# slbouknight/accelerated-ray-tracer

Measured on AMD Instinct MI355X. Metric: Mrays/s, 1200x800 random scene @ 500 spp (frame ms in ms_per_step), higher is better.
Workload: dtype f32

## Files before the change

accelerated-ray-tracer_amd/__init__.py:

```python
from __future__ import annotations

import collections
import ctypes as C
import os
import subprocess

import numpy as np

PKG_DIR = os.path.dirname(os.path.realpath(__file__))
REPO_ROOT = os.path.dirname(PKG_DIR)
LIB_DIR = os.path.join(PKG_DIR, "lib")
RT_LIB_PATH = os.environ.get("RT_LIB_OVERRIDE") or os.path.join(LIB_DIR, "librt_mi355x.so")
HOST_LIB_PATH = os.environ.get("RTW_LIB_OVERRIDE") or os.path.join(LIB_DIR, "librtw_host.so")


class RtError(RuntimeError):
    pass


class RtCamera(C.Structure):
    _fields_ = [("origin", C.c_float * 3), ("lower_left_corner", C.c_float * 3), ("horizontal", C.c_float * 3),
                ("vertical", C.c_float * 3), ("u", C.c_float * 3), ("v", C.c_float * 3), ("lens_radius", C.c_float),
                ("pad", C.c_float), ("time0", C.c_double), ("time1", C.c_double)]

# ... 497 lines not shown
        except Exception:
            pass


def _frame_buffers(color):
    bufs = _Buffers(isinstance(color, np.ndarray), "color", _initialised_device)
    if not (bufs.on_host or hasattr(color, "data_ptr")):
        raise bufs.wrong_kind("color", "a numpy array")
    if color.ndim != 3 or color.shape[2] != 3 or color.shape[0] < 1 or color.shape[1] < 1:
        raise ValueError(f"color: shape {tuple(color.shape)}, expected (ny, nx, 3)")
    ny, nx = int(color.shape[0]), int(color.shape[1])
    if nx * ny >= 1 << 31:
        raise ValueError("frame too large")
    return bufs, nx, ny


_initialised_device = None


def init(device: int = 0) -> None:
    global _initialised_device
    _check(rt_lib().rt_init(device), "rt_init")
    _initialised_device = device


def set_option(key: str, value: int) -> None:
    _check(rt_lib().rt_set_option(key.encode(), int(value)), f"rt_set_option({key})")


def reset_options() -> None:
    _check(rt_lib().rt_reset_options(), "rt_reset_options")


def denoise_workspace_bytes(nx: int, ny: int) -> int:
    return int(rt_lib().rt_denoise_workspace_bytes(int(nx), int(ny)))


def denoise(color, albedo=None, normal=None, depth=None, *, iterations=DENOISE_DEFAULTS["iterations"],
            sigma_color=None, color_floor=DENOISE_DEFAULTS["color_floor"],
            normal_sharpness=DENOISE_DEFAULTS["normal_sharpness"], sigma_depth=DENOISE_DEFAULTS["sigma_depth"], demodulate=None,
            out=None, workspace=None, stream=0, blocking=True, variance=None, variance_out=None,
            sigma_variance=DENOISE_VARIANCE_DEFAULTS["sigma_variance"], variance_floor=DENOISE_VARIANCE_DEFAULTS["variance_floor"]):
    if variance is None:
        if variance_out is not None:
            raise ValueError("variance_out needs variance")
        if sigma_color is None:
            sigma_color = DENOISE_DEFAULTS["sigma_color"]
    else:
        if sigma_color is not None and float(sigma_color) != 0:
            raise ValueError("sigma_color must be left out or 0 with a variance: the variance factor replaces the colour factor")
        sigma_color = 0.0
        sigma_variance, variance_floor = float(sigma_variance), float(variance_floor)
        if not (np.isfinite(sigma_variance) and np.float32(1e-6) <= np.float32(sigma_variance) <= np.float32(1e6)):
            raise ValueError("sigma_variance must be in [1e-6, 1e6]")
        if not (np.isfinite(variance_floor) and 0 < np.float32(variance_floor) < np.inf):
            raise ValueError("variance_floor must be finite and positive")
    bufs, nx, ny = _frame_buffers(color)
    for k, v, lo, hi in (("iterations", iterations, 1, 8), ("normal_sharpness", normal_sharpness, 0, 10)):
        if isinstance(v, bool) or not isinstance(v, (int, np.integer)) or not lo <= int(v) <= hi:
            raise ValueError(f"{k} must be an integer in {lo}..{hi}")
    sigma_color, color_floor, sigma_depth = float(sigma_color), float(color_floor), float(sigma_depth)
    for k, v in (("sigma_color", sigma_color), ("sigma_depth", sigma_depth)):
        if not (v == 0 or (np.isfinite(v) and np.float32(1e-6) <= np.float32(v) <= np.float32(1e6))):
            raise ValueError(f"{k} must be 0 or in [1e-6, 1e6]")
    if sigma_color > 0 and not (np.isfinite(color_floor) and 0 < np.float32(color_floor) < np.inf):
        raise ValueError("color_floor must be finite and positive")
# ... 349 lines not shown
    def spheres(self) -> np.ndarray:
        out = np.zeros(self.host.desc.n_spheres, SPHERE_DTYPE)
        _check(rt_lib().rt_scene_get_spheres(self._p, out.ctypes.data, len(out)), "rt_scene_get_spheres")
        return out

    def instances(self) -> np.ndarray:
        out = np.zeros(self.host.desc.n_instances, INSTANCE_DTYPE)
        _check(rt_lib().rt_scene_get_instances(self._p, out.ctypes.data, len(out)), "rt_scene_get_instances")
        return out

    def quads(self) -> np.ndarray:
        out = np.zeros(self.host.desc.n_quads, QUAD_DTYPE)
        _check(rt_lib().rt_scene_get_quads(self._p, out.ctypes.data, len(out)), "rt_scene_get_quads")
        return out

    def debug_quads(self):
        quads, boxes = np.zeros(self.host.desc.n_quads, QUAD_DTYPE), np.zeros(self.host.desc.n_boxes, np.int32)
        _check(rt_lib().rt_debug_scene_quads(self._p, quads.ctypes.data if len(quads) else None, len(quads),
                                             boxes.ctypes.data if len(boxes) else None, len(boxes)), "rt_debug_scene_quads")
        return quads, boxes

    COST_MAP_STATES = ("none", "exact", "stale")

    def cost_map(self):
        L = rt_lib()
        info = (C.c_int32 * 4)()
        _check(L.rt_debug_cost_map(self._p, None, 0, info), "rt_debug_cost_map")
        if info[0] == 0:
            return "none", None, int(info[3])
        out = np.zeros((int(info[2]), int(info[1])), np.uint32)
        _check(L.rt_debug_cost_map(self._p, out.ctypes.data, out.size, info), "rt_debug_cost_map")
        return self.COST_MAP_STATES[info[0]], out, int(info[3])

    def set_cost_map(self, costs) -> None:
        a = np.ascontiguousarray(costs, np.uint32)
        _check(rt_lib().rt_debug_set_cost_map(self._p, a.ctypes.data, a.size), "rt_debug_set_cost_map")

    def render(self, frame: RtFrameDesc, out=None, stream: int = 0, blocking: bool = True):
        L = rt_lib()
        rows = L.rt_frame_local_rows(C.byref(frame))
        if rows < 0:
            raise RtError("bad row partition")
        stats = RtStats()
        if out is None:
            out = np.empty((rows, frame.nx, 3), np.float32)
        if isinstance(out, np.ndarray):
            assert out.dtype == np.float32 and out.size == rows * frame.nx * 3 and out.flags["C_CONTIGUOUS"]
            _check(L.rt_render(self._p, C.byref(frame), out.ctypes.data, 0, stream, 1, C.byref(stats)), "rt_render")
            return out, stats
        _check(L.rt_render(self._p, C.byref(frame), C.c_void_p(int(out)), 1, stream, 1 if blocking else 0, C.byref(stats)), "rt_render")
        return None, stats

    def _ray_buffers(self, origins, directions):
        bufs = _Buffers(isinstance(origins, np.ndarray), "origins", self.device)
        if not (bufs.on_host or hasattr(origins, "data_ptr")):
            raise bufs.wrong_kind("origins", "a numpy array")
        if origins.ndim != 2 or origins.shape[1] != 3:
            raise ValueError(f"origins: shape {tuple(origins.shape)}, expected (N, 3)")
        if directions is None:
            raise ValueError("directions are required")
        return bufs, int(origins.shape[0])

    def trace(self, origins, directions, times=None, tmin: float = 0.001, tmax=None, any_hit: bool = False, record: bool = False,
              stream=None):
        import torch
        if any_hit and record:
# ... 463 lines not shown
```

accelerated-ray-tracer_amd/csrc/rt_abi.hip:

```cpp
#include <hip/hip_runtime.h>

#include <algorithm>
#include <cfloat>
#include <utility>
#include <cmath>
#include <functional>
#include <cstdio>
#include <cstring>
#include <string>
#include <vector>

#include "../../include/rt_abi.h"
#include "rt_call_buffers.h"
#include "rt_device.h"
#include "rt_refit_host.h"

namespace {

struct device_info {
    bool ready = false;
    int num_cu = 256;
    size_t lds_per_cu = 160 * 1024;
};
enum { RT_MAX_DEVICES = 16 };
device_info g_devices[RT_MAX_DEVICES];
int g_device = -1;
int g_last_hip_error = 0;
std::string g_detail;

struct rt_options {
    int kernel = RT_KERNEL_STAGED;
    int lds_mode = -1;
    int steps_per_trip = 12;
    int shade_threshold = 0;
    int wg_per_cu = 0;
    int threads = 0;
    int leaf_threshold = 8;
    int diel_threshold = 2;
    int box_threshold = 8;
    int medium_threshold = 16;
    int newpath_threshold = 0;
    int sparse_stride = 8;
    int split_samples = 16;
    int tier_auto = 1;
    int tier_kernel = 1;
    int prior = 1;
    int resplit_samples = 0;
    int presplit_samples = 0;
    int tier1_factor_x10 = 45;
    int tier1_pixels = 1536;
    int cost_smooth_percent = 0;
    int tier1_depth = 3;
    int heavy_factor_x10 = 20;
    int sparse_factor_x10 = 40;
    int heavy_max_tiles = 0;
    int semi_stride = -1;
    int sparse_priority = 3;
    int tier_priority = 1;
    int semi_priority = 1;
    int handoff = 1;
    int handoff_scan = 1;
    int handoff_poll_us = 1000;
    int handoff_pixels = -1;
    int sparse_eager = 0;
    int sparse_work_percent = 5;
    int sparse_wg_percent = 35;
    int bvh_collapse = 3;
    int scan_nodes = 24;
    int multi_force_rccl = 0;
    int lpt = 1;
    int cost_map = 1;
    int trace_lds = -1;
    int trace_tree = 1;
    int radiance_lds = -1;
    int aov_lds = -1;
    int aov_through_lds = -1;
    int denoise_lds = -1;
    int upscale_lds = -1;
    int adaptive_tier = -1;
};
rt_options g_opt;
unsigned long long g_opt_epoch = 0;

#define HIPCHK(expr)                                                                  \
    do {                                                                              \
        hipError_t e_ = (expr);                                                       \
        if (e_ != hipSuccess) {                                                       \
            g_last_hip_error = (int)e_;                                               \
            char buf_[512];                                                           \
            snprintf(buf_, sizeof(buf_), "HIP error = %u at %s:%d '%s' (%s)", (unsigned)e_, __FILE__, __LINE__, #expr, \
                     hipGetErrorString(e_));                                          \
            g_detail = buf_;                                                          \
            return RT_ERR_HIP;                                                        \
        }                                                                             \
    } while (0)
#define RT_TRY(expr) do { const rt_status st_ = (expr); if (st_ != RT_OK) return st_; } while (0)
// ... 37 lines not shown
        if (guarded && !all.empty()) (void)hipStreamSynchronize(stream);
        for (void* p : all) (void)hipFree(p);
    }
    void guard(hipStream_t st) { stream = st; guarded = true; }
    void settled() { guarded = false; }
    hipError_t get(void** p, size_t bytes) { const hipError_t e = hipMalloc(p, bytes ? bytes : 1); if (e == hipSuccess) all.push_back(*p); return e; }
    rt_status finish(bool wait) { if (wait) HIPCHK(hipStreamSynchronize(stream)); settled(); return RT_OK; }
};

}

rt_status rt_internal_scene_create_on(int device, const rt_scene_desc* d, rt_scene** out);

struct rt_scene {
    int device = 0;
    rt_scene_dev dev;
    std::vector<void*> allocs;
    bool spheres_only = false, need_uv = false;
    int tex_level = 0;
    size_t node_bytes = 0, sphere_bytes = 0, shade_bytes = 0;
    double walk_tests_before = 0, walk_tests_after = 0;
    unsigned long long* d_ray_counter = nullptr;
    unsigned int* d_work_counter = nullptr;
    float* d_fb = nullptr;
    size_t d_fb_floats = 0;
    unsigned int* d_tile_cost = nullptr;
    unsigned int* d_tile_order = nullptr;
    rt_pixel_state* d_state = nullptr;
    unsigned long long* d_heavy_list = nullptr;
    unsigned int* d_heavy_pixels = nullptr;
    size_t tile_capacity = 0, pixel_capacity = 0;
    unsigned long long* d_handoff = nullptr;
    size_t handoff_capacity = 0;
    rt_rank_info* d_rank = nullptr;
    unsigned int* d_cal_cost = nullptr;
    int cal_nx = 0, cal_ny = 0;
    struct cost_map_key {
        int32_t nx = 0, ny = 0, tile_rows = 0, tile_first = 0, tile_stride = 0, local_rows = 0, kernel_variant = 0;
        bool operator==(const cost_map_key& o) const {
            return nx == o.nx && ny == o.ny && tile_rows == o.tile_rows && tile_first == o.tile_first && tile_stride == o.tile_stride &&
                   local_rows == o.local_rows && kernel_variant == o.kernel_variant;
        }
    };
    struct cost_map_state {
        unsigned int* d = nullptr;
        size_t capacity = 0;
        bool valid = false, pending = false;
        cost_map_key key, last_key;
        bool have_last_key = false;
        unsigned long long scene_epoch = 0, opt_epoch = 0, total = 0;
        int last_parts = 0;
    } cost_map;
    unsigned long long scene_epoch = 0;
    hipStream_t tier_stream = nullptr;
    hipEvent_t ev_fork[4] = {nullptr, nullptr, nullptr, nullptr}, ev_join[4] = {nullptr, nullptr, nullptr, nullptr};
    bool ranked_frame = false;
    hipEvent_t ev_start = nullptr, ev_stop = nullptr;
    bool frame_pending = false;
    hipStream_t pending_stream = nullptr;
    rt_stats pending_stats;
    rt_pixel_state* d_adapt_state = nullptr;
    float* d_adapt_half = nullptr;
    uint32_t* d_adapt_list[2] = {nullptr, nullptr};
    unsigned long long* d_adapt_queue = nullptr;
    int32_t* d_adapt_spp = nullptr;
    uint32_t* d_adapt_count = nullptr;
// ... 402 lines not shown

const char* rt_strerror(rt_status s) {
    switch (s) {
    case RT_OK: return "ok";
    case RT_ERR_INVALID: return "invalid argument or malformed scene description";
    case RT_ERR_NO_DEVICE: return "no gfx950 HIP device";
    case RT_ERR_HIP: return "HIP runtime error";
    case RT_ERR_UNSUPPORTED: return "unsupported scene construct";
    default: return "unknown status";
    }
}
int rt_last_hip_error(void) { return g_last_hip_error; }
const char* rt_last_error_detail(void) { return g_detail.c_str(); }

rt_status rt_set_option(const char* key, int value) {
    if (!key) return invalid("null option key");
    ++g_opt_epoch;
    const std::string k(key);
    if (k == "kernel") { if (value != RT_KERNEL_PIXEL && value != RT_KERNEL_STAGED) return invalid("kernel: 0 (pixel) or 3 (staged)"); g_opt.kernel = value; }
    else if (k == "leaf_threshold") { if (value < 1 || value > 64) return invalid("leaf_threshold: 1..64"); g_opt.leaf_threshold = value; }
    else if (k == "box_threshold") { if (value < 1 || value > 64) return invalid("box_threshold: 1..64"); g_opt.box_threshold = value; }
    else if (k == "medium_threshold") { if (value < 1 || value > 64) return invalid("medium_threshold: 1..64"); g_opt.medium_threshold = value; }
    else if (k == "diel_threshold") { if (value < 1 || value > 64) return invalid("diel_threshold: 1..64"); g_opt.diel_threshold = value; }
    else if (k == "newpath_threshold") { if (value < 0 || value > 64) return invalid("newpath_threshold: 0 (by kernel family) or 1..64"); g_opt.newpath_threshold = value; }
    else if (k == "sparse_stride") { if (value != 0 && value != 2 && value != 4 && value != 8 && value != 16 && value != 32 && value != 64) return invalid("sparse_stride: 0, 2, 4, ... 64"); g_opt.sparse_stride = value; }
    else if (k == "sparse_factor_x10") { if (value < 10 || value > 1000) return invalid("sparse_factor_x10: 10..1000"); g_opt.sparse_factor_x10 = value; }
    else if (k == "heavy_factor_x10") { if (value < 10 || value > 1000) return invalid("heavy_factor_x10: 10..1000"); g_opt.heavy_factor_x10 = value; }
    else if (k == "tier_auto") { if (value < 0 || value > 1) return invalid("tier_auto: 0 or 1"); g_opt.tier_auto = value; }
    else if (k == "tier_kernel") { if (value < 0 || value > 1) return invalid("tier_kernel: 0 or 1"); g_opt.tier_kernel = value; }
    else if (k == "handoff") { if (value < 0 || value > 1) return invalid("handoff: 0 or 1"); g_opt.handoff = value; }
    else if (k == "handoff_scan") { if (value < 0 || value > 1) return invalid("handoff_scan: 0 or 1"); g_opt.handoff_scan = value; }
    else if (k == "handoff_poll_us") { if (value < 1 || value > 1000000) return invalid("handoff_poll_us: 1..1000000"); g_opt.handoff_poll_us = value; }
    else if (k == "handoff_pixels") { if (value < -1 || value > (1 << 24)) return invalid("handoff_pixels: -1 (auto) or 0..16777216"); g_opt.handoff_pixels = value; }
    else if (k == "prior") { if (value < 0 || value > 1) return invalid("prior: 0 or 1"); g_opt.prior = value; }
    else if (k == "presplit_samples") { if (value < 0 || value > 4096) return invalid("presplit_samples: 0..4096"); g_opt.presplit_samples = value; }
    else if (k == "resplit_samples") { if (value < 0 || value > 65536) return invalid("resplit_samples: 0..65536"); g_opt.resplit_samples = value; }
    else if (k == "split_samples") { if (value < 1 || value > 4096) return invalid("split_samples: 1..4096"); g_opt.split_samples = value; }
    else if (k == "tier1_factor_x10") { if (value < 10 || value > 10000) return invalid("tier1_factor_x10: 10..10000"); g_opt.tier1_factor_x10 = value; }
    else if (k == "cost_smooth_percent") { if (value < 0 || value > 100) return invalid("cost_smooth_percent: 0..100"); g_opt.cost_smooth_percent = value; }
    else if (k == "tier1_depth") { if (value < 1 || value > 64) return invalid("tier1_depth: 1..64"); g_opt.tier1_depth = value; }
    else if (k == "tier1_pixels") { if (value < 0 || value > 65536) return invalid("tier1_pixels: 0..65536"); g_opt.tier1_pixels = value; }
    else if (k == "semi_stride") { if (value != -1 && value != 0 && value != 1 && value != 2 && value != 4 && value != 8) return invalid("semi_stride: -1 (by kernel family), 0, 1, 2, 4 or 8"); g_opt.semi_stride = value; }
    else if (k == "sparse_eager") { if (value < 0 || value > 1) return invalid("sparse_eager: 0 or 1"); g_opt.sparse_eager = value; }
    else if (k == "tier_priority") { if (value < 0 || value > 3) return invalid("tier_priority: 0..3"); g_opt.tier_priority = value; }
    else if (k == "semi_priority") { if (value < 0 || value > 3) return invalid("semi_priority: 0..3"); g_opt.semi_priority = value; }
    else if (k == "sparse_priority") { if (value < 0 || value > 3) return invalid("sparse_priority: 0..3"); g_opt.sparse_priority = value; }
    else if (k == "sparse_work_percent") { if (value < 0 || value > 100) return invalid("sparse_work_percent: 0..100"); g_opt.sparse_work_percent = value; }
    else if (k == "sparse_wg_percent") { if (value < 1 || value > 100) return invalid("sparse_wg_percent: 1..100"); g_opt.sparse_wg_percent = value; }
    else if (k == "heavy_max_tiles") { if (value < 0 || value > 4096) return invalid("heavy_max_tiles: 0..4096"); g_opt.heavy_max_tiles = value; }
    else if (k == "bvh_collapse") { if (value < 0 || value > 3) return invalid("bvh_collapse: 0..3 (read by rt_scene_create)"); g_opt.bvh_collapse = value; }
    else if (k == "scan_nodes") { if (value < 0 || value > 64) return invalid("scan_nodes: 0..64"); g_opt.scan_nodes = value; }
    else if (k == "multi_force_rccl") { if (value < 0 || value > 1) return invalid("multi_force_rccl: 0 or 1"); g_opt.multi_force_rccl = value; }
    else if (k == "cost_map") { if (value < 0 || value > 1) return invalid("cost_map: 0 or 1"); g_opt.cost_map = value; }
    else if (k == "lpt") { if (value < 0 || value > 1) return invalid("lpt: 0 or 1"); g_opt.lpt = value; }
    else if (k == "threads") { if (value != 0 && (value < 64 || value > 768 || (value % 64))) return invalid("threads: 0 (per kernel family) or a multiple of 64 up to 768 (512 for the lean spheres-only kernels)"); g_opt.threads = value; }
    else if (k == "lds_mode") { if (value < -1 || value > 4) return invalid("lds_mode: -1..4"); g_opt.lds_mode = value; }
    else if (k == "steps_per_trip") { if (value < 1 || value > 64) return invalid("steps_per_trip: 1..64"); g_opt.steps_per_trip = value; }
    else if (k == "shade_threshold") { if (value < 0 || value > 64) return invalid("shade_threshold: 0 (by the launch's load) or 1..64"); g_opt.shade_threshold = value; }
    else if (k == "trace_lds") { if (value < -1 || value > 2) return invalid("trace_lds: -1 (auto) .. 2"); g_opt.trace_lds = value; }
    else if (k == "radiance_lds") { if (value < -1 || value > 2) return invalid("radiance_lds: -1 (auto) .. 2"); g_opt.radiance_lds = value; }
    else if (k == "aov_lds") { if (value < -1 || value > 2) return invalid("aov_lds: -1 (auto) .. 2"); g_opt.aov_lds = value; }
    else if (k == "aov_through_lds") { if (value < -1 || value > 2) return invalid("aov_through_lds: -1 (auto) .. 2"); g_opt.aov_through_lds = value; }
    else if (k == "denoise_lds") { if (value < -1 || value > 1) return invalid("denoise_lds: -1 (auto), 0 (direct) or 1 (staged)"); g_opt.denoise_lds = value; }
    else if (k == "upscale_lds") { if (value < -1 || value > 1) return invalid("upscale_lds: -1 (auto), 0 (direct) or 1 (staged)"); g_opt.upscale_lds = value; }
    else if (k == "trace_tree") { if (value < 0 || value > 1) return invalid("trace_tree: 0 (reference tree) or 1 (walk array)"); g_opt.trace_tree = value; }
    else if (k == "adaptive_tier") { if (value < -1 || value > 1) return invalid("adaptive_tier: -1 (auto), 0 (main kernel) or 1 (tier kernel)"); g_opt.adaptive_tier = value; }
    else if (k == "wg_per_cu") { if (value < 0 || value > 8) return invalid("wg_per_cu: 0 (per kernel family) .. 8"); g_opt.wg_per_cu = value; }
    else return invalid("unknown option");
    return RT_OK;
}

rt_status rt_scene_destroy(rt_scene* s) {
    if (!s) return RT_OK;
    (void)use_device(s->device);
    for (void* p : s->allocs) (void)hipFree(p);
    if (s->d_ray_counter) (void)hipFree(s->d_ray_counter);
    if (s->d_work_counter) (void)hipFree(s->d_work_counter);
    if (s->d_fb) (void)hipFree(s->d_fb);
    if (s->d_tile_cost) (void)hipFree(s->d_tile_cost);
    if (s->d_tile_order) (void)hipFree(s->d_tile_order);
    if (s->d_state) (void)hipFree(s->d_state);
    if (s->d_heavy_list) (void)hipFree(s->d_heavy_list);
    if (s->d_heavy_pixels) (void)hipFree(s->d_heavy_pixels);
    if (s->d_rank) (void)hipFree(s->d_rank);
    if (s->d_handoff) (void)hipFree(s->d_handoff);
    if (s->d_cal_cost) (void)hipFree(s->d_cal_cost);
    if (s->cost_map.d) (void)hipFree(s->cost_map.d);
    for (void* p : {s->refit.block, (void*)s->refit.d_indices, (void*)s->refit.d_records}) if (p) (void)hipFree(p);
    for (void* p : {(void*)s->d_adapt_state, (void*)s->d_adapt_half, (void*)s->d_adapt_list[0], (void*)s->d_adapt_list[1], (void*)s->d_adapt_queue,
                    (void*)s->d_adapt_spp, (void*)s->d_adapt_count, (void*)s->d_adapt_rank, (void*)s->d_var_acc})
        if (p) (void)hipFree(p);
    for (hipEvent_t e : s->adapt_events) (void)hipEventDestroy(e);
    if (s->tier_stream) (void)hipStreamDestroy(s->tier_stream);
    for (int k = 0; k < 4; ++k) { if (s->ev_fork[k]) (void)hipEventDestroy(s->ev_fork[k]); if (s->ev_join[k]) (void)hipEventDestroy(s->ev_join[k]); }
    if (s->ev_start) (void)hipEventDestroy(s->ev_start);
    if (s->ev_stop) (void)hipEventDestroy(s->ev_stop);
    delete s;
    return RT_OK;
}

namespace {
rt_status measure_pass_counts(rt_scene* s, const rt_node* d_tree, int n_tree, std::vector<double>& pass, double& rays, std::vector<float>* sample = nullptr, uint32_t sample_stride = 0, bool keep_cost = false) {
    const rt_camera& c = s->dev.camera;
    const double hw = sqrt((double)c.horizontal[0] * c.horizontal[0] + (double)c.horizontal[1] * c.horizontal[1] + (double)c.horizontal[2] * c.horizontal[2]);
    const double vh = sqrt((double)c.vertical[0] * c.vertical[0] + (double)c.vertical[1] * c.vertical[1] + (double)c.vertical[2] * c.vertical[2]);
    double aspect = (hw > 0 && vh > 0) ? hw / vh : 1.0;
    if (!(aspect > 0.05 && aspect < 20.0)) aspect = 1.0;
    int nx = aspect >= 1.0 ? 256 : (int)(256 * aspect + 0.5), ny = aspect >= 1.0 ? (int)(256 / aspect + 0.5) : 256;
    if (nx < 8) nx = 8;
    if (ny < 8) ny = 8;
    const int n = n_tree;
    rt_scene_dev dev = s->dev;
    dev.nodes_ref = d_tree; dev.n_nodes_ref = n_tree;
    unsigned int* d_pass = nullptr;
    unsigned int* d_cost = nullptr;
    float* d_fb = nullptr;
    HIPCHK(hipMalloc((void**)&d_pass, (size_t)n * sizeof(unsigned int)));
    hipError_t e = hipMalloc((void**)&d_fb, (size_t)nx * ny * 3 * sizeof(float));
// ... 1303 lines not shown
}

rt_status rt_reproject(const rt_reproject_desc* d, int buffers_on_device, void* stream_v, int blocking) {
    return reproject_impl(d, nullptr, nullptr, nullptr, "rt_reproject", buffers_on_device, stream_v, blocking);
}

rt_status rt_reproject_moving(const rt_reproject_desc* d, const rt_reproject_motion_desc* m, int buffers_on_device, void* stream_v, int blocking) {
    if (!m) return invalid("rt_reproject_moving: null motion description");
    return reproject_impl(d, m, nullptr, nullptr, "rt_reproject_moving", buffers_on_device, stream_v, blocking);
}

rt_status rt_reproject_instances(const rt_reproject_desc* d, const rt_reproject_motion_desc* m, const rt_reproject_instance_desc* im,
                                 int buffers_on_device, void* stream_v, int blocking) {
    if (!m) return invalid("rt_reproject_instances: null motion description");
    if (!im) return invalid("rt_reproject_instances: null instance description");
    return reproject_impl(d, m, im, nullptr, "rt_reproject_instances", buffers_on_device, stream_v, blocking);
}

rt_status rt_reproject_quads(const rt_reproject_desc* d, const rt_reproject_motion_desc* m, const rt_reproject_instance_desc* im,
                             const rt_reproject_quad_desc* qm, int buffers_on_device, void* stream_v, int blocking) {
    if (!m) return invalid("rt_reproject_quads: null motion description");
    if (!im) return invalid("rt_reproject_quads: null instance description");
    if (!qm) return invalid("rt_reproject_quads: null quad description");
    return reproject_impl(d, m, im, qm, "rt_reproject_quads", buffers_on_device, stream_v, blocking);
}

rt_status rt_debug_handoff(rt_scene* s, unsigned long long* out2) {
    if (!s || !out2) return invalid("null argument");
    RT_TRY(use_device(s->device));
    HIPCHK(hipMemcpy(out2, s->d_ray_counter + 28, 2 * sizeof(unsigned long long), hipMemcpyDeviceToHost));
    return RT_OK;
}

rt_status rt_debug_counters(rt_scene* s, unsigned long long* out16) {
    if (!s || !out16) return invalid("null argument");
    RT_TRY(use_device(s->device));
    HIPCHK(hipMemcpy(out16, s->d_ray_counter + 1, 16 * sizeof(unsigned long long), hipMemcpyDeviceToHost));
    return RT_OK;
}
rt_status rt_debug_stage_cycles(rt_scene* s, unsigned long long* out10) {
    if (!s || !out10) return invalid("null argument");
    RT_TRY(use_device(s->device));
    HIPCHK(hipMemcpy(out10, s->d_ray_counter + 17, 10 * sizeof(unsigned long long), hipMemcpyDeviceToHost));
    return RT_OK;
}
rt_status rt_debug_wave_ends(rt_scene* s, unsigned long long* out, int n) {
    if (!s || !out || n < 0 || n > 2 * RT_DIAG_BINS) return invalid("bad argument");
    RT_TRY(use_device(s->device));
    HIPCHK(hipMemcpy(out, s->d_ray_counter + RT_DIAG_HIST_SLOT, (size_t)n * sizeof(unsigned long long), hipMemcpyDeviceToHost));
    return RT_OK;
}
rt_status rt_debug_wave_last(rt_scene* s, unsigned long long* out, int n_waves) {
    if (!s || !out || n_waves < 0 || n_waves > RT_DIAG_MAX_WAVES) return invalid("bad argument");
    RT_TRY(use_device(s->device));
    HIPCHK(hipMemcpy(out, s->d_ray_counter + RT_DIAG_WAVE_SLOT, (size_t)2 * n_waves * sizeof(unsigned long long), hipMemcpyDeviceToHost));
    return RT_OK;
}

namespace {
enum { RANK_PARAM_WORDS = 20, RANK_INFO_WORDS = 13 };
static_assert(sizeof(rt_rank_info) == RANK_INFO_WORDS * 4, "rt_debug_rank / rt_debug_rank_info copy rt_rank_info as 13 words");
}

rt_status rt_debug_rank(const uint32_t* cost, const uint32_t* tile_cost, uint64_t rays, const uint32_t* params, uint32_t* tile_order,
                        uint32_t* cost_out, uint32_t* heavy_pixels, uint32_t* info13) {
    if (!cost || !tile_cost || !params || !tile_order || !cost_out || !heavy_pixels || !info13) return invalid("rt_debug_rank: null argument");
// ... 495 lines not shown
    dim3 grid = ml.grid;
    const dim3 block = ml.block;
    const int per_cu_resident = ml.per_cu_resident;

    bool tier_possible = false;
    unsigned tier_grid = 0;
    int tier_waves_per_main_wg = 0;
    tier_room room = {false, 0, 0, 0};
    if (kernel == RT_KERNEL_STAGED && (g_opt.tier_kernel || g_opt.handoff) && s->dev.leaf_lo != nullptr) {
        size_t budget;
        if (lean_family) {
            const size_t used = (size_t)per_cu_resident * (ml.lds_bytes + 512);
            budget = g_lds_per_cu > used + 1024 ? g_lds_per_cu - used - 1024 : 0;
        } else {
            const unsigned tier_wgs_per_slot = block.x / RT_TIER_THREADS > 0 ? block.x / RT_TIER_THREADS : 1u;
            budget = (g_lds_per_cu / (size_t)per_cu_resident - 1024) / tier_wgs_per_slot;
            tier_waves_per_main_wg = (int)(tier_wgs_per_slot * (RT_TIER_THREADS / 64));
        }
        room = plan_tier_room(s, budget);
        if (room.fits) {
            tier_possible = g_opt.tier_kernel && lds_mode != 4 && g_opt.tier1_pixels > 0;
            tier_grid = lean_family ? (unsigned)(2 * g_num_cu) : (unsigned)(g_num_cu * per_cu_resident) * (unsigned)(tier_waves_per_main_wg / (RT_TIER_THREADS / 64)) / 2u;
            if (tier_grid < 1u) tier_grid = 1u;
        }
    }
    fp.tier_lds_scene = room.lds_scene;
    const size_t tier_lds = room.lds;
    const unsigned tail_grid = room.fits && g_opt.handoff && (lds_mode != 4 || g_opt.handoff_scan) ? room.tail_grid : 0u;

    HIPCHK(hipEventRecord(s->ev_start, stream));
    const size_t n_tiles = (size_t)g.tiles_x * (size_t)g.tiles_y;
    const size_t n_pixels = g.n_pixels;
    s->ranked_frame = false;
    HIPCHK(hipMemsetAsync(s->d_ray_counter, 0, 256, stream));
    int part_index = 0;
    auto launch_part = [&](const rt_frame_params& q, dim3 grid_q, bool ranked) -> rt_status {
        HIPCHK(hipMemsetAsync(s->d_work_counter, 0, RT_WORK_COUNTER_BYTES, stream));
        const bool tiers = ranked && tier_possible;
        const int pi = part_index++ & 3;
        if (tiers) {
            HIPCHK(hipEventRecord(s->ev_fork[pi], stream));
            HIPCHK(hipStreamWaitEvent(s->tier_stream, s->ev_fork[pi], 0));
            HIPCHK(launch_tier(s, q, dim3(tier_grid), tier_lds, s->tier_stream));
            HIPCHK(hipEventRecord(s->ev_join[pi], s->tier_stream));
        }
        HIPCHK(launch_render(kernel, lds_mode, s, q, grid_q, block, ml.lds_bytes, stream));
        if (q.handoff_queue) {
            rt_frame_params t = q;
            t.tail_mode = 1;
            HIPCHK(launch_tier(s, t, dim3(tail_grid), tier_lds, stream));
        }
        if (tiers) HIPCHK(hipStreamWaitEvent(stream, s->ev_join[pi], 0));
        return RT_OK;
    };
    if (win) {
        fp.state_in = win_begin > 0 ? win->d_state : nullptr; fp.state_out = win->d_state;
        fp.sample_begin = win_begin; fp.sample_end = win_end; fp.store_parked = 1;
    } else if (g_opt.lpt && kernel == RT_KERNEL_STAGED && f->ns >= 2 * g_opt.split_samples && n_tiles >= 64 && n_pixels < (1ull << 31)) {
        RT_TRY(grow_ranked_buffers(s, n_tiles, n_pixels));
        rt_scene::cost_map_state& cm = s->cost_map;
        rt_scene::cost_map_key key;
        key.nx = f->nx; key.ny = f->ny; key.tile_rows = f->tile_rows; key.tile_first = f->tile_first; key.tile_stride = f->tile_stride;
        key.local_rows = g.local_rows; key.kernel_variant = out.kernel_variant;
        if (g_opt.cost_map && cm.capacity < n_pixels) { cm.valid = false; RT_TRY(grow(cm.d, cm.capacity, n_pixels)); }
        const bool map_read = lean_family || !tier_possible;
        const bool map_usable = g_opt.cost_map && g_opt.prior && map_read && cm.valid && cm.total > 0 && cm.key == key;
        const bool map_exact = map_usable && cm.scene_epoch == s->scene_epoch && cm.opt_epoch == g_opt_epoch;
        if (tail_grid > 0) {
            RT_TRY(grow(s->d_handoff, s->handoff_capacity, (size_t)g_num_cu * (size_t)per_cu_resident * (size_t)block.x));
            fp.handoff_queue = s->d_handoff; fp.handoff_cap = (uint32_t)s->handoff_capacity; fp.handoff_state = s->d_state;
            fp.handoff_poll_ticks = g_opt.handoff_poll_us * 100;
            const size_t tail_waves = (size_t)tail_grid * (RT_TIER_THREADS / 64);
            const size_t cap_px = n_pixels / 8;
            fp.handoff_pixels = g_opt.handoff_pixels >= 0 ? g_opt.handoff_pixels : (int32_t)(6 * tail_waves < cap_px ? 6 * tail_waves : cap_px);
        }
        const unsigned max_grid = (unsigned)(g_num_cu * per_cu_resident);
        const tier_sizes e = effective_tier_sizes((double)n_pixels / ((double)max_grid * (double)block.x), lean_family, g_opt);
        auto rank_pixels = [&](rt_frame_params& q, dim3& grid_q, const unsigned long long* total) -> rt_status {
            rt_rank_params rp;
            memset(&rp, 0, sizeof(rp));
            rp.state = s->d_state; rp.tile_cost = s->d_tile_cost; rp.tile_order = s->d_tile_order; rp.ray_counter = total;
            rp.heavy_list = s->d_heavy_list; rp.heavy_pixels = s->d_heavy_pixels; rp.info = s->d_rank;
            rp.n_pixels = (uint32_t)n_pixels; rp.n_tiles = (uint32_t)n_tiles; rp.heavy_cap = RT_HEAVY_CAP;
            rp.max_grid = max_grid; rp.waves_per_wg = block.x / 64u;
            rp.normal_need = (uint32_t)((q.work_items + block.x - 1) / block.x);
            rp.sparse_stride = (g_opt.sparse_stride > 0 && block.x >= 64) ? g_opt.sparse_stride : 0;
            rp.semi_stride = g_opt.semi_stride >= 0 ? g_opt.semi_stride : (lean_family ? 1 : 0);
            rp.sparse_percent = e.sparse_percent;
            rp.sparse_work_percent = e.work_percent;
            rp.tier_possible = tier_possible ? 1 : 0;
            rp.tier1_pixels = e.tier1_pixels; rp.tier1_depth = e.tier1_depth;
            rp.tier_wgs_cap = (int32_t)tier_grid; rp.tier_waves_per_main_wg = tier_waves_per_main_wg;
            rp.nx = f->nx; rp.smooth_percent = g_opt.cost_smooth_percent;
            rp.heavy_factor = (float)e.heavy_factor / 10.0f; rp.sparse_factor = (float)e.sparse_factor / 10.0f; rp.tier1_factor = (float)e.tier1_factor / 10.0f;
            HIPCHK(rt_launch_rank(rp, stream));
            q.tile_order = s->d_tile_order; q.heavy_pixels = s->d_heavy_pixels; q.rank = s->d_rank;
            unsigned total_wgs = rp.normal_need + (rp.sparse_stride > 0 ? max_grid * (unsigned)e.sparse_percent / 100u : 0u);
            if (tier_waves_per_main_wg > 0 && tier_possible) total_wgs = max_grid;
            if (total_wgs > max_grid) total_wgs = max_grid;
            if (total_wgs < 1u) total_wgs = 1u;
            grid_q = dim3(total_wgs);
            return RT_OK;
        };
        auto ranked_part = [&](int begin, int end) -> rt_status {
            rt_frame_params q = fp;
            dim3 grid_q = grid;
            q.sample_begin = begin; q.sample_end = end;
// ... 309 lines not shown
```

accelerated-ray-tracer_amd/csrc/rt_rank.hip:

```cpp
#include <hip/hip_runtime.h>
#include <stdint.h>

#include "rt_device.h"

namespace {

enum { RANK_THREADS = 1024, RANK_BUCKETS = 2048 };

__device__ unsigned int wg_reduce_max(unsigned int v, unsigned int* scratch) {
    if (threadIdx.x == 0) *scratch = 0u;
    __syncthreads();
    atomicMax(scratch, v);
    __syncthreads();
    const unsigned int r = *scratch;
    __syncthreads();
    return r;
}
__device__ unsigned int wg_reduce_min(unsigned int v, unsigned int* scratch) {
    if (threadIdx.x == 0) *scratch = 0xFFFFFFFFu;
    __syncthreads();
    atomicMin(scratch, v);
    __syncthreads();
    const unsigned int r = *scratch;
    __syncthreads();
    return r;
}

template <class Key, class Val>
__device__ void wg_bucket_sort_desc(unsigned int n, Key key, Val value, unsigned int* out, unsigned int* hist, unsigned int* scratch,
                                    unsigned int* hi_out = nullptr, unsigned long long* span_out = nullptr) {
    unsigned int lo = 0xFFFFFFFFu, hi = 0u;
    for (unsigned int i = threadIdx.x; i < n; i += blockDim.x) { const unsigned int k = key(i); lo = k < lo ? k : lo; hi = k > hi ? k : hi; }
    hi = wg_reduce_max(hi, scratch);
    lo = wg_reduce_min(lo, scratch);
    const unsigned long long span = (unsigned long long)(hi >= lo ? hi - lo : 0u) + 1ull;
    for (unsigned int b = threadIdx.x; b <= RANK_BUCKETS; b += blockDim.x) hist[b] = 0u;
// ... 150 lines not shown
        const int t = lrow / pp.tile_rows;
        const int j = (pp.tile_first + t * pp.tile_stride) * pp.tile_rows + (lrow - t * pp.tile_rows);
        const int ci = min(pp.cal_nx - 1, (int)(((long long)i * pp.cal_nx) / pp.nx)), cj = min(pp.cal_ny - 1, (int)(((long long)j * pp.cal_ny) / pp.ny));
        for (int dj = -1; dj <= 1; ++dj)
            for (int di = -1; di <= 1; ++di) {
                const int x = ci + di, y = cj + dj;
                if (x < 0 || y < 0 || x >= pp.cal_nx || y >= pp.cal_ny) continue;
                const unsigned int c = pp.cal_cost[(size_t)y * pp.cal_nx + x];
                est = c > est ? c : est;
            }
        pp.state[p].cost = est;
        atomicAdd(&pp.tile_cost[(lrow >> 3) * pp.tiles_x + (i >> 3)], est);
    }
    unsigned long long sum = est;
    for (int off = 32; off > 0; off >>= 1) sum += __shfl_down(sum, off, 64);
    if ((threadIdx.x & 63) == 0 && sum) atomicAdd(pp.total, sum);
}

__global__ void rt_prior_map_kernel(rt_prior_params pp) {
    const unsigned int p = blockIdx.x * blockDim.x + threadIdx.x;
    const unsigned int n = (unsigned int)pp.local_rows * (unsigned int)pp.nx;
    unsigned int est = 0u;
    if (p < n) {
        const unsigned int lrow = p / (unsigned int)pp.nx, i = p - lrow * (unsigned int)pp.nx;
        est = pp.cal_cost[p] & 0x7FFFFFFFu;
        pp.state[p].cost = est;
        atomicAdd(&pp.tile_cost[(lrow >> 3) * (unsigned int)pp.tiles_x + (i >> 3)], est);
    }
    unsigned long long sum = est;
    for (int off = 32; off > 0; off >>= 1) sum += __shfl_down(sum, off, 64);
    if ((threadIdx.x & 63) == 0 && sum) atomicAdd(pp.total, sum);
}

}

hipError_t rt_launch_prior(const rt_prior_params& pp, hipStream_t st) {
    const unsigned int n = (unsigned int)pp.local_rows * (unsigned int)pp.nx;
    hipLaunchKernelGGL(rt_prior_kernel, dim3((n + 255u) / 256u), dim3(256), 0, st, pp);
    return hipGetLastError();
}

hipError_t rt_launch_prior_map(const rt_prior_params& pp, hipStream_t st) {
    const unsigned int n = (unsigned int)pp.local_rows * (unsigned int)pp.nx;
    hipLaunchKernelGGL(rt_prior_map_kernel, dim3((n + 255u) / 256u), dim3(256), 0, st, pp);
    return hipGetLastError();
}

hipError_t rt_launch_rank(const rt_rank_params& rp, hipStream_t st) {
    hipLaunchKernelGGL(rt_rank_tiles_kernel, dim3(1), dim3(RANK_THREADS), 0, st, rp);
    hipError_t e = hipGetLastError();
    if (e != hipSuccess) return e;
    hipLaunchKernelGGL(rt_collect_heavy_kernel, dim3((rp.n_pixels + 255u) / 256u), dim3(256), 0, st, rp);
    if ((e = hipGetLastError()) != hipSuccess) return e;
    hipLaunchKernelGGL(rt_rank_heavy_kernel, dim3(1), dim3(RANK_THREADS), 0, st, rp);
    return hipGetLastError();
}
```

Baseline: 15110.

## Order handoff tail queue by estimated remaining work before tail launch

Adds a two-kernel histogram/scatter pass that sorts handoff queue entries into descending buckets of estimated remaining cost (samples to go times rays per done sample). The tail kernel then serves the longest-remaining pixels first, an LPT-style order meant to shorten the straggler tail. On the lean family it also doubles the default handoff pixels per wave. It costs two extra small kernel launches, a scratch memset per part, and extra buffers. Debug entry points and Python helpers are added to inspect the ordering.

```diff
diff --git a/accelerated-ray-tracer_amd/__init__.py b/accelerated-ray-tracer_amd/__init__.py
--- a/accelerated-ray-tracer_amd/__init__.py
+++ b/accelerated-ray-tracer_amd/__init__.py
@@ -553,6 +553,41 @@
     _check(rt_lib().rt_reset_options(), "rt_reset_options")
 
 
+HANDOFF_SUB_BITS = 2
+HANDOFF_BUCKETS = 1 + 64 * (1 << HANDOFF_SUB_BITS)
+HANDOFF_ORDER_MIN_PER_WAVE, HANDOFF_ORDER_MAX_PER_WAVE = 2, 32
+
+
+def handoff_order_key(entries, costs, sample_begin: int, sample_end: int):
+    e = np.asarray(entries, np.uint64)
+    nxt = (e >> np.uint64(32)).astype(np.int64)
+    rays = (np.asarray(costs, np.uint32) & np.uint32(0x7FFFFFFF)).astype(np.int64)
+    to_go, done = np.maximum(int(sample_end) - nxt, 0), np.maximum(nxt - int(sample_begin), 0)
+    return np.array([int(t) * (int(r) + 1) // (int(d) + 1) for t, r, d in zip(to_go, rays, done)], dtype=object)
+
+
+def handoff_order_bucket(keys):
+    out = np.zeros(len(keys), np.int64)
+    for i, k in enumerate(keys):
+        k = int(k)
+        if k > 0:
+            e = k.bit_length() - 1
+            m = (k >> (e - HANDOFF_SUB_BITS) if e >= HANDOFF_SUB_BITS else k << (HANDOFF_SUB_BITS - e)) & ((1 << HANDOFF_SUB_BITS) - 1)
+            out[i] = 1 + (e << HANDOFF_SUB_BITS) + m
+    return out
+
+
+def debug_order_handoff(entries, costs, sample_begin: int, sample_end: int, tail_waves: int):
+    e, c = np.ascontiguousarray(entries, np.uint64), np.ascontiguousarray(costs, np.uint32)
+    assert e.ndim == 1 and c.shape == e.shape
+    out, overrun = np.zeros(len(e), np.uint64), C.c_uint32(0xFFFFFFFF)
+    L = rt_lib()
+    L.rt_debug_order_handoff.argtypes = [C.c_void_p, C.c_void_p, C.c_int64, C.c_int32, C.c_int32, C.c_int32, C.c_void_p, C.POINTER(C.c_uint32)]
+    _check(L.rt_debug_order_handoff(e.ctypes.data if len(e) else None, c.ctypes.data if len(e) else None, len(e), int(sample_begin), int(sample_end),
+                                    int(tail_waves), out.ctypes.data if len(e) else None, C.byref(overrun)), "rt_debug_order_handoff")
+    return out, int(overrun.value)
+
+
 def denoise_workspace_bytes(nx: int, ny: int) -> int:
     return int(rt_lib().rt_denoise_workspace_bytes(int(nx), int(ny)))
 
@@ -968,6 +1003,17 @@
         _check(L.rt_debug_cost_map(self._p, out.ctypes.data, out.size, info), "rt_debug_cost_map")
         return self.COST_MAP_STATES[info[0]], out, int(info[3])
 
+    def handoff_queue(self):
+        L = rt_lib()
+        L.rt_debug_handoff_queue.argtypes = [C.c_void_p, C.c_void_p, C.c_void_p, C.c_void_p, C.c_int64, C.POINTER(C.c_int64)]
+        info = (C.c_int64 * 4)()
+        _check(L.rt_debug_handoff_queue(self._p, None, None, None, 0, info), "rt_debug_handoff_queue")
+        n = int(info[0])
+        entries, costs, served = np.zeros(n, np.uint64), np.zeros(n, np.uint32), np.zeros(n, np.uint64)
+        if n:
+            _check(L.rt_debug_handoff_queue(self._p, entries.ctypes.data, costs.ctypes.data, served.ctypes.data, n, info), "rt_debug_handoff_queue")
+        return entries, costs, served, dict(ordered=bool(info[1]), min=int(info[2]), max=int(info[3]))
+
     def set_cost_map(self, costs) -> None:
         a = np.ascontiguousarray(costs, np.uint32)
         _check(rt_lib().rt_debug_set_cost_map(self._p, a.ctypes.data, a.size), "rt_debug_set_cost_map")
diff --git a/accelerated-ray-tracer_amd/csrc/rt_abi.hip b/accelerated-ray-tracer_amd/csrc/rt_abi.hip
--- a/accelerated-ray-tracer_amd/csrc/rt_abi.hip
+++ b/accelerated-ray-tracer_amd/csrc/rt_abi.hip
@@ -13,6 +13,7 @@
 #include "../../include/rt_abi.h"
 #include "rt_call_buffers.h"
 #include "rt_device.h"
+#include "rt_handoff_order.h"
 #include "rt_refit_host.h"
 
 namespace {
@@ -62,6 +63,7 @@
     int handoff_scan = 1;
     int handoff_poll_us = 1000;
     int handoff_pixels = -1;
+    int handoff_order = 1;
     int sparse_eager = 0;
     int sparse_work_percent = 5;
     int sparse_wg_percent = 35;
@@ -165,6 +167,12 @@
     size_t tile_capacity = 0, pixel_capacity = 0;
     unsigned long long* d_handoff = nullptr;
     size_t handoff_capacity = 0;
+    unsigned long long* d_handoff_ordered = nullptr;
+    size_t handoff_ordered_capacity = 0;
+    unsigned int* d_handoff_scratch = nullptr;
+    size_t handoff_scratch_capacity = 0;
+    bool tail_ordered = false;
+    uint32_t tail_order_min = 0, tail_order_max = 0;
     rt_rank_info* d_rank = nullptr;
     unsigned int* d_cal_cost = nullptr;
     int cal_nx = 0, cal_ny = 0;
@@ -633,6 +641,7 @@
     else if (k == "handoff_scan") { if (value < 0 || value > 1) return invalid("handoff_scan: 0 or 1"); g_opt.handoff_scan = value; }
     else if (k == "handoff_poll_us") { if (value < 1 || value > 1000000) return invalid("handoff_poll_us: 1..1000000"); g_opt.handoff_poll_us = value; }
     else if (k == "handoff_pixels") { if (value < -1 || value > (1 << 24)) return invalid("handoff_pixels: -1 (auto) or 0..16777216"); g_opt.handoff_pixels = value; }
+    else if (k == "handoff_order") { if (value < 0 || value > 1) return invalid("handoff_order: 0 or 1"); g_opt.handoff_order = value; }
     else if (k == "prior") { if (value < 0 || value > 1) return invalid("prior: 0 or 1"); g_opt.prior = value; }
     else if (k == "presplit_samples") { if (value < 0 || value > 4096) return invalid("presplit_samples: 0..4096"); g_opt.presplit_samples = value; }
     else if (k == "resplit_samples") { if (value < 0 || value > 65536) return invalid("resplit_samples: 0..65536"); g_opt.resplit_samples = value; }
@@ -685,6 +694,8 @@
     if (s->d_heavy_pixels) (void)hipFree(s->d_heavy_pixels);
     if (s->d_rank) (void)hipFree(s->d_rank);
     if (s->d_handoff) (void)hipFree(s->d_handoff);
+    if (s->d_handoff_ordered) (void)hipFree(s->d_handoff_ordered);
+    if (s->d_handoff_scratch) (void)hipFree(s->d_handoff_scratch);
     if (s->d_cal_cost) (void)hipFree(s->d_cal_cost);
     if (s->cost_map.d) (void)hipFree(s->cost_map.d);
     for (void* p : {s->refit.block, (void*)s->refit.d_indices, (void*)s->refit.d_records}) if (p) (void)hipFree(p);
@@ -2054,6 +2065,75 @@
     return RT_OK;
 }
 
+rt_status rt_debug_handoff_queue(rt_scene* s, unsigned long long* entries, uint32_t* costs, unsigned long long* served, int64_t cap, int64_t* info4) {
+    if (!s || !info4 || cap < 0 || (cap > 0 && (!entries || !costs || !served))) return invalid("rt_debug_handoff_queue: bad argument");
+    if (s->frame_pending) return invalid("rt_debug_handoff_queue: a frame is pending (rt_frame_finish first)");
+    info4[0] = 0; info4[1] = s->tail_ordered ? 1 : 0; info4[2] = s->tail_order_min; info4[3] = s->tail_order_max;
+    int64_t* const count_out = info4;
+    if (!s->d_handoff || !s->d_state || !s->ranked_frame) return RT_OK;
+    RT_TRY(use_device(s->device));
+    unsigned int pushed = 0;
+    HIPCHK(hipMemcpy(&pushed, s->d_work_counter + RT_WC_PUSHED, sizeof(pushed), hipMemcpyDeviceToHost));
+    const size_t count = pushed < s->handoff_capacity ? pushed : s->handoff_capacity;
+    *count_out = (int64_t)count;
+    const size_t n = count < (size_t)cap ? count : (size_t)cap;
+    if (n == 0) return RT_OK;
+    HIPCHK(hipMemcpy(entries, s->d_handoff, n * sizeof(unsigned long long), hipMemcpyDeviceToHost));
+    HIPCHK(hipMemcpy(served, s->tail_ordered ? s->d_handoff_ordered : s->d_handoff, n * sizeof(unsigned long long), hipMemcpyDeviceToHost));
+    std::vector<rt_pixel_state> h_state(s->pixel_capacity);
+    HIPCHK(hipMemcpy(h_state.data(), s->d_state, h_state.size() * sizeof(rt_pixel_state), hipMemcpyDeviceToHost));
+    for (size_t i = 0; i < n; ++i) {
+        const uint32_t pix = (uint32_t)entries[i];
+        costs[i] = pix < h_state.size() ? h_state[pix].cost : 0u;
+    }
+    return RT_OK;
+}
+
+enum { ORDER_SEAM_SLACK = 3 };
+rt_status rt_debug_order_handoff(const unsigned long long* entries, const uint32_t* costs, int64_t n, int32_t sample_begin, int32_t sample_end,
+                                 int32_t tail_waves, unsigned long long* out, uint32_t* overrun_out) {
+    if (!overrun_out) return invalid("rt_debug_order_handoff: null argument");
+    if (n < 0 || n > (1ll << 24) || (n > 0 && (!entries || !costs || !out))) return invalid("rt_debug_order_handoff: n must be 0 .. 2^24 and the arrays non-null");
+    if (sample_begin < 0 || sample_end < sample_begin) return invalid("rt_debug_order_handoff: bad sample range");
+    if (tail_waves < 1 || tail_waves > (1 << 20)) return invalid("rt_debug_order_handoff: tail_waves must be 1 .. 2^20");
+    for (int64_t i = 0; i < n; ++i)
+        if ((int64_t)(uint32_t)entries[i] >= n) return invalid("rt_debug_order_handoff: an entry's pixel is not below n");
+    RT_TRY(use_device(g_device));
+    call_memory mem;
+    rt_handoff_order_params hp;
+    memset(&hp, 0, sizeof(hp));
+    const size_t most = (size_t)RT_HANDOFF_ORDER_MAX_PER_WAVE * (size_t)tail_waves;
+    hp.cap = (uint32_t)n; hp.min_items = (uint32_t)(RT_HANDOFF_ORDER_MIN_PER_WAVE * tail_waves); hp.max_items = (uint32_t)(most < (size_t)n ? most : (size_t)n);
+    hp.cost_begin = sample_begin; hp.sample_end = sample_end;
+    unsigned long long *d_queue = nullptr, *d_ordered = nullptr;
+    rt_pixel_state* d_state = nullptr;
+    unsigned int* d_pushed = nullptr;
+    const size_t scratch_bytes = rt_handoff_order_scratch_words(hp.max_items) * sizeof(unsigned int);
+    HIPCHK(mem.get((void**)&d_queue, (size_t)(n + ORDER_SEAM_SLACK) * sizeof(unsigned long long)));
+    HIPCHK(mem.get((void**)&d_ordered, (size_t)(n + ORDER_SEAM_SLACK) * sizeof(unsigned long long)));
+    HIPCHK(mem.get((void**)&d_state, (size_t)(n + 1) * sizeof(rt_pixel_state)));
+    HIPCHK(mem.get((void**)&d_pushed, sizeof(unsigned int)));
+    HIPCHK(mem.get((void**)&hp.scratch, scratch_bytes));
+    std::vector<rt_pixel_state> h_state((size_t)n + 1);
+    for (int64_t i = 0; i < n; ++i) h_state[(size_t)i].cost = costs[i];
+    const unsigned int h_pushed = (unsigned int)n + ORDER_SEAM_SLACK;
+    HIPCHK(hipMemset(d_queue, 0, (size_t)(n + ORDER_SEAM_SLACK) * sizeof(unsigned long long)));
+    if (n > 0) HIPCHK(hipMemcpy(d_queue, entries, (size_t)n * sizeof(unsigned long long), hipMemcpyHostToDevice));
+    HIPCHK(hipMemcpy(d_state, h_state.data(), h_state.size() * sizeof(rt_pixel_state), hipMemcpyHostToDevice));
+    HIPCHK(hipMemset(d_ordered, 0xFF, (size_t)(n + ORDER_SEAM_SLACK) * sizeof(unsigned long long)));
+    HIPCHK(hipMemcpy(d_pushed, &h_pushed, sizeof(h_pushed), hipMemcpyHostToDevice));
+    HIPCHK(hipMemset(hp.scratch, 0, scratch_bytes));
+    hp.queue = d_queue; hp.ordered = d_ordered; hp.state = d_state; hp.pushed = d_pushed;
+    HIPCHK(rt_launch_handoff_order(hp, nullptr));
+    HIPCHK(hipDeviceSynchronize());
+    if (n > 0) HIPCHK(hipMemcpy(out, d_ordered, (size_t)n * sizeof(unsigned long long), hipMemcpyDeviceToHost));
+    unsigned long long spare[ORDER_SEAM_SLACK];
+    HIPCHK(hipMemcpy(spare, d_ordered + n, sizeof(spare), hipMemcpyDeviceToHost));
+    *overrun_out = 0u;
+    for (const unsigned long long w : spare) *overrun_out += w != ~0ull ? 1u : 0u;
+    return RT_OK;
+}
+
 rt_status rt_debug_counters(rt_scene* s, unsigned long long* out16) {
     if (!s || !out16) return invalid("null argument");
     RT_TRY(use_device(s->device));
@@ -2615,10 +2695,14 @@
     const size_t n_tiles = (size_t)g.tiles_x * (size_t)g.tiles_y;
     const size_t n_pixels = g.n_pixels;
     s->ranked_frame = false;
+    s->tail_ordered = false; s->tail_order_min = s->tail_order_max = 0;
     HIPCHK(hipMemsetAsync(s->d_ray_counter, 0, 256, stream));
     int part_index = 0;
+    bool order_tail = false;
+    uint32_t order_min = 0, order_max = 0;
     auto launch_part = [&](const rt_frame_params& q, dim3 grid_q, bool ranked) -> rt_status {
         HIPCHK(hipMemsetAsync(s->d_work_counter, 0, RT_WORK_COUNTER_BYTES, stream));
+        if (order_tail && q.handoff_queue) HIPCHK(hipMemsetAsync(s->d_handoff_scratch, 0, RT_HANDOFF_BUCKETS * sizeof(unsigned int), stream));
         const bool tiers = ranked && tier_possible;
         const int pi = part_index++ & 3;
         if (tiers) {
@@ -2631,6 +2715,16 @@
         if (q.handoff_queue) {
             rt_frame_params t = q;
             t.tail_mode = 1;
+            if (order_tail) {
+                rt_handoff_order_params hp;
+                memset(&hp, 0, sizeof(hp));
+                hp.queue = q.handoff_queue; hp.ordered = s->d_handoff_ordered; hp.state = q.handoff_state;
+                hp.pushed = q.work_counter + RT_WC_PUSHED; hp.scratch = s->d_handoff_scratch;
+                hp.cap = q.handoff_cap; hp.min_items = order_min; hp.max_items = order_max;
+                hp.cost_begin = (q.state_in && !q.fresh) ? 0 : q.sample_begin; hp.sample_end = q.sample_end;
+                HIPCHK(rt_launch_handoff_order(hp, stream));
+                t.handoff_queue = s->d_handoff_ordered;
+            }
             HIPCHK(launch_tier(s, t, dim3(tail_grid), tier_lds, stream));
         }
         if (tiers) HIPCHK(hipStreamWaitEvent(stream, s->ev_join[pi], 0));
@@ -2655,7 +2749,17 @@
             fp.handoff_poll_ticks = g_opt.handoff_poll_us * 100;
             const size_t tail_waves = (size_t)tail_grid * (RT_TIER_THREADS / 64);
             const size_t cap_px = n_pixels / 8;
-            fp.handoff_pixels = g_opt.handoff_pixels >= 0 ? g_opt.handoff_pixels : (int32_t)(6 * tail_waves < cap_px ? 6 * tail_waves : cap_px);
+            const size_t per_wave = (g_opt.handoff_order && lean_family) ? 12 : 6;
+            fp.handoff_pixels = g_opt.handoff_pixels >= 0 ? g_opt.handoff_pixels : (int32_t)(per_wave * tail_waves < cap_px ? per_wave * tail_waves : cap_px);
+            if (g_opt.handoff_order) {
+                const size_t most = (size_t)RT_HANDOFF_ORDER_MAX_PER_WAVE * tail_waves;
+                order_min = (uint32_t)(RT_HANDOFF_ORDER_MIN_PER_WAVE * tail_waves);
+                order_max = (uint32_t)(most < s->handoff_capacity ? most : s->handoff_capacity);
+                RT_TRY(grow(s->d_handoff_ordered, s->handoff_ordered_capacity, s->handoff_capacity));
+                RT_TRY(grow(s->d_handoff_scratch, s->handoff_scratch_capacity, rt_handoff_order_scratch_words(order_max)));
+                order_tail = true;
+                s->tail_ordered = true; s->tail_order_min = order_min; s->tail_order_max = order_max;
+            }
         }
         const unsigned max_grid = (unsigned)(g_num_cu * per_cu_resident);
         const tier_sizes e = effective_tier_sizes((double)n_pixels / ((double)max_grid * (double)block.x), lean_family, g_opt);
diff --git a/accelerated-ray-tracer_amd/csrc/rt_handoff_order.h b/accelerated-ray-tracer_amd/csrc/rt_handoff_order.h
--- /dev/null
+++ b/accelerated-ray-tracer_amd/csrc/rt_handoff_order.h
@@ -0,0 +1,29 @@
+#pragma once
+#include <hip/hip_runtime.h>
+#include <stdint.h>
+
+#include "rt_device.h"
+
+enum { RT_HANDOFF_SUB_BITS = 2,
+       RT_HANDOFF_BUCKETS = 1 + 64 * (1 << RT_HANDOFF_SUB_BITS),
+       RT_HANDOFF_ORDER_THREADS = 256,
+       RT_HANDOFF_ORDER_MIN_PER_WAVE = 2,
+       RT_HANDOFF_ORDER_MAX_PER_WAVE = 32 };
+
+struct rt_handoff_order_params {
+    const unsigned long long* queue;
+    unsigned long long* ordered;
+    const rt_pixel_state* state;
+    const unsigned int* pushed;
+    unsigned int* scratch;
+    uint32_t cap;
+    uint32_t min_items, max_items;
+    int32_t cost_begin;
+    int32_t sample_end;
+};
+
+inline size_t rt_handoff_order_scratch_words(uint32_t max_items) {
+    const size_t wgs = ((size_t)max_items + RT_HANDOFF_ORDER_THREADS - 1) / RT_HANDOFF_ORDER_THREADS;
+    return (size_t)RT_HANDOFF_BUCKETS * (wgs + 1);
+}
+hipError_t rt_launch_handoff_order(const rt_handoff_order_params& hp, hipStream_t st);
diff --git a/accelerated-ray-tracer_amd/csrc/rt_rank.hip b/accelerated-ray-tracer_amd/csrc/rt_rank.hip
--- a/accelerated-ray-tracer_amd/csrc/rt_rank.hip
+++ b/accelerated-ray-tracer_amd/csrc/rt_rank.hip
@@ -2,6 +2,7 @@
 #include <stdint.h>
 
 #include "rt_device.h"
+#include "rt_handoff_order.h"
 
 namespace {
 
@@ -218,6 +219,72 @@
     if ((threadIdx.x & 63) == 0 && sum) atomicAdd(pp.total, sum);
 }
 
+__device__ __forceinline__ unsigned int handoff_count(const rt_handoff_order_params& hp) {
+    const unsigned int pushed = *hp.pushed;
+    return pushed < hp.cap ? pushed : hp.cap;
+}
+__device__ __forceinline__ unsigned int handoff_bucket(const rt_handoff_order_params& hp, unsigned long long entry) {
+    const int next = (int)(entry >> 32);
+    const unsigned long long rays = hp.state[(uint32_t)entry].cost & 0x7FFFFFFFu;
+    const unsigned long long to_go = next < hp.sample_end ? (unsigned long long)(hp.sample_end - next) : 0ull;
+    const unsigned long long done = next > hp.cost_begin ? (unsigned long long)(next - hp.cost_begin) : 0ull;
+    const unsigned long long key = to_go * (rays + 1ull) / (done + 1ull);
+    if (key == 0ull) return 0u;
+    const int e = 63 - __clzll((long long)key);
+    const unsigned int m = (unsigned int)(e >= RT_HANDOFF_SUB_BITS ? key >> (e - RT_HANDOFF_SUB_BITS) : key << (RT_HANDOFF_SUB_BITS - e)) & ((1u << RT_HANDOFF_SUB_BITS) - 1u);
+    return 1u + ((unsigned int)e << RT_HANDOFF_SUB_BITS) + m;
+}
+
+__global__ void __launch_bounds__(RT_HANDOFF_ORDER_THREADS) rt_handoff_hist_kernel(rt_handoff_order_params hp) {
+    __shared__ unsigned int h[RT_HANDOFF_BUCKETS];
+    const unsigned int count = handoff_count(hp);
+    if (count < hp.min_items || count > hp.max_items || blockIdx.x * RT_HANDOFF_ORDER_THREADS >= count) return;
+    for (unsigned int b = threadIdx.x; b < RT_HANDOFF_BUCKETS; b += RT_HANDOFF_ORDER_THREADS) h[b] = 0u;
+    __syncthreads();
+    const unsigned int i = blockIdx.x * RT_HANDOFF_ORDER_THREADS + threadIdx.x;
+    if (i < count) atomicAdd(&h[handoff_bucket(hp, hp.queue[i])], 1u);
+    __syncthreads();
+    unsigned int* wg_start = hp.scratch + (size_t)RT_HANDOFF_BUCKETS * (blockIdx.x + 1u);
+    for (unsigned int b = threadIdx.x; b < RT_HANDOFF_BUCKETS; b += RT_HANDOFF_ORDER_THREADS) {
+        const unsigned int c = h[b];
+        wg_start[b] = c ? atomicAdd(&hp.scratch[b], c) : 0u;
+    }
+}
+
+__global__ void __launch_bounds__(RT_HANDOFF_ORDER_THREADS) rt_handoff_scatter_kernel(rt_handoff_order_params hp) {
+    __shared__ unsigned int total[RT_HANDOFF_BUCKETS], start[RT_HANDOFF_BUCKETS];
+    const unsigned int count = handoff_count(hp);
+    if (count < hp.min_items || count > hp.max_items) {
+        for (unsigned int i = blockIdx.x * RT_HANDOFF_ORDER_THREADS + threadIdx.x; i < count; i += gridDim.x * RT_HANDOFF_ORDER_THREADS) hp.ordered[i] = hp.queue[i];
+        return;
+    }
+    if (blockIdx.x * RT_HANDOFF_ORDER_THREADS >= count) return;
+    for (unsigned int b = threadIdx.x; b < RT_HANDOFF_BUCKETS; b += RT_HANDOFF_ORDER_THREADS) total[b] = hp.scratch[b];
+    __syncthreads();
+    const unsigned int* wg_start = hp.scratch + (size_t)RT_HANDOFF_BUCKETS * (blockIdx.x + 1u);
+    for (unsigned int b = threadIdx.x; b < RT_HANDOFF_BUCKETS; b += RT_HANDOFF_ORDER_THREADS) {
+        unsigned int above = 0u;
+        for (unsigned int k = b + 1u; k < RT_HANDOFF_BUCKETS; ++k) above += total[k];
+        start[b] = above + wg_start[b];
+    }
+    __syncthreads();
+    const unsigned int i = blockIdx.x * RT_HANDOFF_ORDER_THREADS + threadIdx.x;
+    if (i < count) {
+        const unsigned long long entry = hp.queue[i];
+        hp.ordered[atomicAdd(&start[handoff_bucket(hp, entry)], 1u)] = entry;
+    }
+}
+
+}
+
+hipError_t rt_launch_handoff_order(const rt_handoff_order_params& hp, hipStream_t st) {
+    const unsigned int wgs = (hp.max_items + RT_HANDOFF_ORDER_THREADS - 1u) / RT_HANDOFF_ORDER_THREADS;
+    const dim3 grid(wgs > 0u ? wgs : 1u);
+    hipLaunchKernelGGL(rt_handoff_hist_kernel, grid, dim3(RT_HANDOFF_ORDER_THREADS), 0, st, hp);
+    const hipError_t e = hipGetLastError();
+    if (e != hipSuccess) return e;
+    hipLaunchKernelGGL(rt_handoff_scatter_kernel, grid, dim3(RT_HANDOFF_ORDER_THREADS), 0, st, hp);
+    return hipGetLastError();
 }
 
 hipError_t rt_launch_prior(const rt_prior_params& pp, hipStream_t st) {
```

After: 15640, median of 6. 1.04x the previous value.
